# voxelmorph/voxelmorph

Measured on NVIDIA H100. Metric: vol-pairs/sec (3D 160x192x224 VxmDense int_steps=7 train step, NCC+Grad, Adam), higher is better.
Workload: dtype bf16 (conv operands) / f32 (accumulate, warp, VecInt, losses)

## Files before the change

### voxelmorph_b200/csrc/conv3d_tc_wgrad2.cu

```cuda
#include <stdlib.h>

#include <type_traits>

#include "tc_common.cuh"

namespace vxm {
namespace tcw {

using namespace vxm::tc;

constexpr int TH = 4, TWR = 32, TUSE = 30;
constexpr int XROWS = (TH + 2) * TWR;
constexpr int GPAD = 16, GROWS = TH * TWR, GSROWS = GROWS + 2 * GPAD;
constexpr int MAXSLOT = 8, NGS = 4;
constexpr int NLOADER = 128, NTHREADS = 384;

struct Wgrad2Args {
  const __nv_bfloat16* x; int Cx, up, upd;
  const __nv_bfloat16* gz; int Cg;
  float* partial;
  float* bias_partial;
  int B, D, H, W;
  int tiles_h, tiles_w, dchunk, nchunks, nitems, nslot;
  int dbg;
  int xpitch, gpitch;
};

__host__ __device__ inline uint32_t swz(uint32_t off, uint32_t width) { return off ^ (((off >> 7) & (width / 16 - 1)) << 4); }

template <int WIDTH>
__device__ __forceinline__ uint64_t make_desc_mn_swz(uint32_t saddr, uint32_t lbo_bytes) {
  uint64_t d = 0;
  d |= (uint64_t)((saddr >> 4) & 0x3FFF);
  d |= (uint64_t)((lbo_bytes >> 4) & 0x3FFF) << 16;
  d |= (uint64_t)(((8u * WIDTH) >> 4) & 0x3FFF) << 32;
  return d | desc_swizzle(WIDTH);
}

template <int KD, int G, int GOUT, bool KHM = false>
__global__ void __launch_bounds__(NTHREADS, 1) wgrad2_kernel(const Wgrad2Args a) {
  static_assert(!KHM || (KD == 1 && G == 16), "kh-in-M needs a 2-D operand with 16-channel rows");
  constexpr int WA = 2 * G, WG = 2 * GOUT;
  constexpr uint32_t XSLAB = XROWS * WA, GSLAB = GSROWS * WG;
  constexpr int MM = (KD * G > 64) ? 128 : 64;
  constexpr int NN = 3 * GOUT;
  constexpr int NMIRROR = KD == 3 ? 2 : 0, NPADSLAB = KD == 3 ? 1 : 0;
  constexpr int T = KD * 9;
  constexpr int KX = XROWS * (G / 8) / NLOADER, KG = GROWS * (GOUT / 8) / NLOADER;
  static_assert(XROWS * (G / 8) % NLOADER == 0 && GROWS * (GOUT / 8) % NLOADER == 0, "loader tables");
  constexpr int NPART = KHM ? 1 : 2;
  constexpr int NKH = KHM ? 1 : (MM == 128 ? 3 : 2);

  extern __shared__ __align__(1024) uint8_t smem[];
  const int NS = a.nslot;
  uint8_t* s_x = smem;
  uint8_t* s_g = s_x + (size_t)(NS + NMIRROR + NPADSLAB) * XSLAB;
  uint64_t* bars = reinterpret_cast<uint64_t*>(s_g + NGS * GSLAB);
  uint64_t* xfull = bars;
  uint64_t* xempty = bars + MAXSLOT;
  uint64_t* gfull = bars + 2 * MAXSLOT;
  uint64_t* gempty = gfull + NGS;
  float* s_bsum = reinterpret_cast<float*>(bars) + 128;

  const int warp = threadIdx.x >> 5, lane = threadIdx.x & 31;

  for (uint32_t i = threadIdx.x * 16u; i < NGS * GSLAB; i += NTHREADS * 16u) *reinterpret_cast<uint4*>(s_g + i) = make_uint4(0u, 0u, 0u, 0u);
  if (NPADSLAB)
    for (uint32_t i = threadIdx.x * 16u; i < XSLAB; i += NTHREADS * 16u)
      *reinterpret_cast<uint4*>(s_x + (size_t)(NS + NMIRROR) * XSLAB + i) = make_uint4(0u, 0u, 0u, 0u);
  fence_proxy_async();
  if (threadIdx.x == 0) {
    for (int i = 0; i < NS; ++i) { mbar_init(&xfull[i], NLOADER); mbar_init(&xempty[i], 4 * NPART); }
    for (int i = 0; i < NGS; ++i) { mbar_init(&gfull[i], NLOADER); mbar_init(&gempty[i], 4 * NPART); }
    fence_barrier_init();
  }
  __syncthreads();
  const int HW_tiles = a.tiles_h * a.tiles_w;
  const bool has_work = blockIdx.x < a.nitems;

  if (warp >= 8) {
    setmaxnreg_dec<64>();
    const int lt = threadIdx.x - 8 * 32;
    uint32_t xslot = 0, xphase = 1, gslot = 0, gphase = 1;
    const int Dx = a.upd ? a.D >> 1 : a.D, Hx = a.up ? a.H >> 1 : a.H, Wx = a.up ? a.W >> 1 : a.W;
    const int ncx = a.Cx >> 3, ncg = a.Cg >> 3;
    for (int item = blockIdx.x; item < a.nitems; item += gridDim.x) {
      const int wt = item % a.tiles_w, ht = (item / a.tiles_w) % a.tiles_h;
      const int ch = (item / HW_tiles) % a.nchunks, b = item / (HW_tiles * a.nchunks);
      const int h0 = ht * TH, w0 = wt * TUSE, d0 = ch * a.dchunk, d1 = min(d0 + a.dchunk, a.D);
      const int s_begin = KD == 3 ? d0 - 1 : d0, s_end = KD == 3 ? d1 + 1 : d1;
      int soff[KX];
      uint32_t doff[KX];
#pragma unroll
      for (int k = 0; k < KX; ++k) {
        const int id = lt + k * NLOADER;
        const int c8 = id % (G / 8), row = id / (G / 8);
        const int h = h0 - 1 + (row >> 5), w = w0 - 1 + (row & 31);
        doff[k] = swz((uint32_t)row * WA + (uint32_t)c8 * 16u, WA);
        soff[k] = -1;
        if (h >= 0 && h < a.H && w >= 0 && w < a.W && c8 < ncx) soff[k] = ((a.up ? h >> 1 : h) * Wx + (a.up ? w >> 1 : w)) * a.xpitch + c8 * 8;
      }
      int goff[KG];
      uint32_t gdoff[KG];
#pragma unroll
      for (int k = 0; k < KG; ++k) {
        const int id = lt + k * NLOADER;
        const int c8 = id % (GOUT / 8), row = id / (GOUT / 8);
        const int jj = row & 31, h = h0 + (row >> 5), w = w0 - 1 + jj;
        gdoff[k] = swz((uint32_t)(GPAD + row) * WG + (uint32_t)c8 * 16u, WG);
        goff[k] = -1;
        if (jj >= 1 && jj <= TUSE && h < a.H && w < a.W && c8 < ncg) goff[k] = (h * a.W + w) * a.gpitch + c8 * 8;
      }
      for (int ds = s_begin; ds < s_end; ++ds) {
        mbar_wait(&xempty[xslot], xphase);
        uint8_t* slab = s_x + (size_t)xslot * XSLAB;
        const bool dok = ds >= 0 && ds < a.D;
        const __nv_bfloat16* base = a.x + (((size_t)b * Dx + (dok ? (a.upd ? ds >> 1 : ds) : 0)) * Hx * Wx) * a.xpitch;
#pragma unroll
        for (int k = 0; k < KX; ++k) {
          const bool ok = dok && soff[k] >= 0;
          const __nv_bfloat16* src = ok ? base + soff[k] : a.x;
          if (a.dbg & 2) continue;
          cp_async16(slab + doff[k], src, ok ? 16u : 0u);
          if (NMIRROR && xslot < (uint32_t)NMIRROR) cp_async16(slab + (size_t)NS * XSLAB + doff[k], src, ok ? 16u : 0u);
        }
        cp_async_arrive_noinc(&xfull[xslot]);
        if (++xslot == (uint32_t)NS) { xslot = 0; xphase ^= 1; }
        const int dg = KD == 3 ? ds - 1 : ds;
        if (dg >= d0 && dg < d1) {
          mbar_wait(&gempty[gslot], gphase);
          uint8_t* gt = s_g + (size_t)gslot * GSLAB;
          const __nv_bfloat16* baseG = a.gz + (((size_t)b * a.D + dg) * a.H * a.W) * a.gpitch;
#pragma unroll
          for (int k = 0; k < KG; ++k) {
            const bool ok = goff[k] >= 0;
            if (a.dbg & 2) continue;
            cp_async16(gt + gdoff[k], ok ? baseG + goff[k] : a.gz, ok ? 16u : 0u);
          }
          cp_async_arrive_noinc(&gfull[gslot]);
          if (++gslot == NGS) { gslot = 0; gphase ^= 1; }
        }
      }
    }
  } else {
    setmaxnreg_inc<216>();
    const int wg = warp >> 2;
    const int t = threadIdx.x & 127;
    float acc[NKH][NN / 2];
    float* bsum = s_bsum + t * (GOUT + 1);
    if (wg == 0)
#pragma unroll
      for (int c = 0; c < GOUT; ++c) bsum[c] = 0.f;
    const bool do_bias = wg == 0 && a.bias_partial && !(a.dbg & 4);
    uint32_t roff[GOUT / 8];
#pragma unroll
    for (int c8 = 0; c8 < GOUT / 8; ++c8) roff[c8] = swz((uint32_t)(GPAD + t) * WG + (uint32_t)c8 * 16u, WG);
    if (has_work && wg < NPART) {
      const uint32_t x_u32 = smem_u32(s_x), g_u32 = smem_u32(s_g);
      uint32_t wslot = 0, wphase = 0;
      uint32_t hslot = 0;
      uint32_t gs = 0, gph = 0;
      uint32_t acc0 = 0;
      const uint32_t m_off = (MM == 128 && wg == 1) ? 2u * XSLAB : 0u;
      for (int item = blockIdx.x; item < a.nitems; item += gridDim.x) {
        const int ch = (item / HW_tiles) % a.nchunks;
        const int nd = min(ch * a.dchunk + a.dchunk, a.D) - ch * a.dchunk;
        for (int j = 0; j < nd; ++j) {
          const int nwait = (KD == 3 && j == 0) ? 3 : 1;
          for (int q = 0; q < nwait; ++q) {
            mbar_wait(&xfull[wslot], wphase);
            if (++wslot == (uint32_t)NS) { wslot = 0; wphase ^= 1; }
          }
          mbar_wait(&gfull[gs], gph);
          const uint32_t a_start = x_u32 + hslot * XSLAB + m_off;
          const uint32_t b_start = g_u32 + gs * GSLAB + (uint32_t)(GPAD - 1) * WG;
          const uint64_t adesc0 = make_desc_mn_swz<WA>(a_start, KHM ? (uint32_t)(TWR * WA) : (KD == 3 ? XSLAB : 0u));
          const uint64_t bdesc0 = make_desc_mn_swz<WG>(b_start, (uint32_t)WG);
          auto chain = [&](auto nk, int kh0) {
            constexpr int NK = decltype(nk)::value;
            wg_fence();
#pragma unroll
            for (int s = 0; s < NK; ++s) {
#pragma unroll
              for (int i = 0; i < GROWS / 16; ++i) {
                const uint64_t adesc = adesc0 + (uint64_t)((((kh0 + s) * TWR + 16 * i) * WA) >> 4);
                const uint64_t bdesc = bdesc0 + (uint64_t)((16 * i * WG) >> 4);
                Wgmma<NN, 1, 1>::mma(acc[s], adesc, bdesc, i == 0 ? acc0 : 1u);
              }
            }
            wg_commit();
          };
          if (MM == 128 || KHM || wg == 0) chain(std::integral_constant<int, NKH>{}, 0);
          else chain(std::integral_constant<int, 1>{}, 2);
          if (do_bias) {
            const uint8_t* gt = s_g + (size_t)gs * GSLAB;
#pragma unroll
            for (int c8 = 0; c8 < GOUT / 8; ++c8) {
              const uint4 q = *reinterpret_cast<const uint4*>(gt + roff[c8]);
              const __nv_bfloat162* hq = reinterpret_cast<const __nv_bfloat162*>(&q);
#pragma unroll
              for (int e = 0; e < 4; ++e) {
                const float2 f = __bfloat1622float2(hq[e]);
                bsum[c8 * 8 + 2 * e] += f.x;
                bsum[c8 * 8 + 2 * e + 1] += f.y;
              }
            }
          }
          wg_wait<0>();
          if (lane == 0) {
            mbar_arrive(&xempty[hslot]);
            mbar_arrive(&gempty[gs]);
          }
          acc0 = 1u;
          if (++hslot == (uint32_t)NS) hslot = 0;
          if (++gs == NGS) { gs = 0; gph ^= 1; }
        }
        if (KD == 3) {
          if (lane == 0) {
            mbar_arrive(&xempty[hslot]);
            mbar_arrive(&xempty[hslot + 1 == (uint32_t)NS ? 0 : hslot + 1]);
          }
          hslot = hslot + 2 >= (uint32_t)NS ? hslot + 2 - NS : hslot + 2;
        }
      }
    }
    float* part = a.partial + (size_t)blockIdx.x * T * G * GOUT;
    if (!has_work) {
      if (wg == 0)
        for (int i = t; i < T * G * GOUT; i += 128) part[i] = 0.f;
    } else if (wg < NPART) {
      const int w4 = t >> 5, qr = lane >> 2, pc = lane & 3;
#pragma unroll
      for (int s = 0; s < NKH; ++s) {
        const int kh = KHM ? 0 : (MM == 128 ? s : (wg == 0 ? s : 2));
        if (MM != 128 && !KHM && wg == 1 && s > 0) break;
#pragma unroll
        for (int i = 0; i < 2; ++i) {
          const int m = (MM == 128 ? 64 * wg : 0) + 16 * w4 + 8 * i + qr;
          const int kd = KHM ? 0 : m / G, ci = m % G, khm = KHM ? m / G : kh;
          if (kd >= KD || khm >= 3) continue;
#pragma unroll
          for (int jn = 0; jn < NN / 8; ++jn) {
            const int n = 8 * jn + 2 * pc, q = n / GOUT, co = n % GOUT;
            const int tap = (kd * 3 + khm) * 3 + (2 - q);
            *reinterpret_cast<float2*>(part + ((size_t)tap * G + ci) * GOUT + co) = make_float2(acc[s][4 * jn + 2 * i], acc[s][4 * jn + 2 * i + 1]);
          }
        }
      }
    }
    if (wg == 0 && a.bias_partial) {
      named_bar(1, 128);
      if (t < GOUT) {
        float sum = 0.f;
        for (int r2 = 0; r2 < 128; ++r2) sum += s_bsum[r2 * (GOUT + 1) + t];
        a.bias_partial[(size_t)blockIdx.x * GOUT + t] = sum;
      }
    }
  }
}

constexpr int PTH = 2, PTU = 31;
constexpr int PXROWS = (PTH + 1) * TWR, PXR = PXROWS + 8;
constexpr int PGROWS = PTH * TWR;
constexpr uint32_t PXSLAB = PXR * 64, PGSLAB = PGROWS * 64, PGSTAGE = 16 * PGSLAB;
constexpr int PFROWS = 2 * PTH + 1, PFCOLS = 2 * TWR + 1, PFCHUNKS = PFROWS * PFCOLS * 4;
constexpr uint32_t PFSLICE = PFCHUNKS * 16;
constexpr int PNGS = 2, PNSLOT = 4, PMAXSLOT = 8, PNTHREADS = 512;
constexpr size_t PSMEM = (size_t)PNGS * PGSTAGE + 512 + (size_t)PNSLOT * PXSLAB + 3 * PFSLICE + 512 + 128 * 8 * sizeof(float);

struct Wgrad2PolyArgs {
  const __nv_bfloat16* x; int xpitch;
  const __nv_bfloat16* gz; int Cg, gpitch;
  float* partial;
  float* bias_partial;
  int B, D, H, W, Dc, Hc, Wc;
  int tiles_h, tiles_w, dchunk, nchunks, nitems, nslot;
};

__host__ __device__ constexpr int poly_slab(int hl, int ad, int ah, int aw) { return ((hl * 2 + ad) * 2 + ah) * 2 + aw; }

__global__ void __launch_bounds__(PNTHREADS, 1) wgrad2_poly_kernel(const Wgrad2PolyArgs a) {
  extern __shared__ __align__(1024) uint8_t smem[];
  const int NS = a.nslot;
  uint8_t* s_g = smem;
  uint8_t* s_x = s_g + PNGS * PGSTAGE + 512;
  uint8_t* s_f = s_x + (size_t)NS * PXSLAB;
  uint64_t* bars = reinterpret_cast<uint64_t*>(s_f + 3 * PFSLICE);
  uint64_t* xfull = bars;
  uint64_t* xempty = bars + PMAXSLOT;
  uint64_t* gfull = bars + 2 * PMAXSLOT;
  uint64_t* gempty = gfull + PNGS;
  float* s_bsum = reinterpret_cast<float*>(bars) + 128;

  const int warp = threadIdx.x >> 5, lane = threadIdx.x & 31;
  for (uint32_t i = threadIdx.x * 16u; i < (uint32_t)(PNGS * PGSTAGE + 512 + NS * PXSLAB); i += PNTHREADS * 16u)
    *reinterpret_cast<uint4*>(smem + i) = make_uint4(0u, 0u, 0u, 0u);
  fence_proxy_async();
  if (threadIdx.x == 0) {
    for (int i = 0; i < NS; ++i) { mbar_init(&xfull[i], 128); mbar_init(&xempty[i], 12); }
    for (int i = 0; i < PNGS; ++i) { mbar_init(&gfull[i], 128); mbar_init(&gempty[i], 12); }
    fence_barrier_init();
  }
  __syncthreads();
  const int HW_tiles = a.tiles_h * a.tiles_w;
  const bool has_work = blockIdx.x < a.nitems;

  if (warp >= 12) {
    const int lt = threadIdx.x - 12 * 32;
    const int c8 = lt & 3;
    uint32_t xslot = 0, xphase = 1, gslot = 0, gphase = 1;
    float* bsum = s_bsum + lt * 8;
#pragma unroll
    for (int e = 0; e < 8; ++e) bsum[e] = 0.f;
    const bool cok = c8 * 8 < a.Cg;
    for (int item = blockIdx.x; item < a.nitems; item += gridDim.x) {
      const int wt = item % a.tiles_w, ht = (item / a.tiles_w) % a.tiles_h;
      const int ch = (item / HW_tiles) % a.nchunks, b = item / (HW_tiles * a.nchunks);
      const int h0 = ht * PTH, w0 = wt * PTU, d0 = ch * a.dchunk, d1 = min(d0 + a.dchunk, a.Dc + 1);
      constexpr int KX = PXROWS * 4 / 128;
      int soff[KX];
      uint32_t doff[KX];
#pragma unroll
      for (int k = 0; k < KX; ++k) {
        const int row = (lt + k * 128) >> 2;
        const int h = h0 - 1 + row / TWR, w = w0 - 1 + row % TWR;
        doff[k] = swz((uint32_t)row * 64u + (uint32_t)c8 * 16u, 64);
        soff[k] = (h >= 0 && h < a.Hc && w >= 0 && w < a.Wc) ? (h * a.Wc + w) * a.xpitch + c8 * 8 : -1;
      }
      auto load_fine = [&](int f, bool need) {
        if (need) {
          uint8_t* dst = s_f + (size_t)((f + 3) % 3) * PFSLICE;
          const bool fok = f >= 0 && f < a.D;
          for (int idx = lt; idx < PFCHUNKS; idx += 128) {
            const int r = idx / (PFCOLS * 4), rem = idx - r * (PFCOLS * 4), col = rem >> 2, cc = rem & 3;
            const int fh = 2 * h0 - 1 + r, fw = 2 * w0 - 3 + col;
            const bool ok = fok && fh >= 0 && fh < a.H && fw >= 0 && fw < a.W && cc * 8 < a.Cg;
            cp_async16(dst + (size_t)idx * 16, ok ? a.gz + ((((size_t)b * a.D + f) * a.H + fh) * a.W + fw) * a.gpitch + cc * 8 : a.gz,
                       ok ? 16u : 0u);
          }
        }
        cp_async_commit();
      };
      load_fine(2 * d0 - 1, true);
      load_fine(2 * d0, true);
      load_fine(2 * d0 + 1, true);
      for (int s = d0 - 1; s < d1; ++s) {
        mbar_wait(&xempty[xslot], xphase);
        uint8_t* slab = s_x + (size_t)xslot * PXSLAB;
        const bool dok = s >= 0 && s < a.Dc;
        const __nv_bfloat16* base = a.x + ((size_t)b * a.Dc + (dok ? s : 0)) * a.Hc * a.Wc * a.xpitch;
#pragma unroll
        for (int k = 0; k < KX; ++k) {
          const bool ok = dok && soff[k] >= 0;
          cp_async16(slab + doff[k], ok ? base + soff[k] : a.x, ok ? 16u : 0u);
        }
        cp_async_arrive_noinc(&xfull[xslot]);
        if (++xslot == (uint32_t)NS) { xslot = 0; xphase ^= 1; }
        if (s < d0) continue;
        mbar_wait(&gempty[gslot], gphase);
        uint8_t* st = s_g + (size_t)gslot * PGSTAGE;
#pragma unroll 1
        for (int ad = 0; ad < 2; ++ad) {
          cp_async_wait<1>();
          named_bar(1, 128);
#pragma unroll 1
          for (int u = lt >> 2; u < PGROWS; u += 32) {
            const int i = u / TWR, j = u % TWR;
            float g[2][2][8];
#pragma unroll
            for (int q = 0; q < 32; ++q) (&g[0][0][0])[q] = 0.f;
            if (j > 0 && cok) {
#pragma unroll
              for (int kd = 0; kd < 2; ++kd) {
                const int fd = 2 * s - 1 + ad + kd;
                if (fd < 0 || fd >= a.D) continue;
                const uint8_t* fs = s_f + (size_t)((fd + 3) % 3) * PFSLICE;
#pragma unroll
                for (int kh = 0; kh < 3; ++kh) {
                  float f[3][8];
#pragma unroll
                  for (int kw = 0; kw < 3; ++kw) {
                    const uint4 q = *reinterpret_cast<const uint4*>(fs + (size_t)((((2 * i + kh) * PFCOLS) + 2 * j + kw) * 4 + c8) * 16);
                    const __nv_bfloat162* hq = reinterpret_cast<const __nv_bfloat162*>(&q);
#pragma unroll
                    for (int e = 0; e < 4; ++e) {
                      const float2 v = __bfloat1622float2(hq[e]);
                      f[kw][2 * e] = v.x; f[kw][2 * e + 1] = v.y;
                    }
                  }
#pragma unroll
                  for (int ah = 0; ah < 2; ++ah) {
                    if (ah == 0 ? kh == 2 : kh == 0) continue;
#pragma unroll
                    for (int e = 0; e < 8; ++e) {
                      g[ah][0][e] += f[0][e] + f[1][e];
                      g[ah][1][e] += f[1][e] + f[2][e];
                    }
                  }
                }
              }
              if (ad == 1)
#pragma unroll
                for (int e = 0; e < 8; ++e) bsum[e] += g[1][1][e];
            }
            const uint32_t roff = swz((uint32_t)u * 64u + (uint32_t)c8 * 16u, 64);
#pragma unroll
            for (int ah = 0; ah < 2; ++ah)
#pragma unroll
              for (int aw = 0; aw < 2; ++aw) {
                uint32_t hi[4], lo[4];
#pragma unroll
                for (int e = 0; e < 4; ++e) {
                  const float v0 = g[ah][aw][2 * e], v1 = g[ah][aw][2 * e + 1];
                  const __nv_bfloat162 h2 = __floats2bfloat162_rn(v0, v1);
                  const float2 hf = __bfloat1622float2(h2);
                  hi[e] = *reinterpret_cast<const uint32_t*>(&h2);
                  lo[e] = pack_bf16x2(v0 - hf.x, v1 - hf.y);
                }
                *reinterpret_cast<uint4*>(st + (size_t)poly_slab(0, ad, ah, aw) * PGSLAB + roff) = make_uint4(hi[0], hi[1], hi[2], hi[3]);
                *reinterpret_cast<uint4*>(st + (size_t)poly_slab(1, ad, ah, aw) * PGSLAB + roff) = make_uint4(lo[0], lo[1], lo[2], lo[3]);
              }
          }
          named_bar(1, 128);
          load_fine(2 * s + 2 + ad, s + 1 < d1);
        }
        fence_proxy_async();
        mbar_arrive(&gfull[gslot]);
        if (++gslot == PNGS) { gslot = 0; gphase ^= 1; }
      }
    }
    if (a.bias_partial) {
      named_bar(1, 128);
      if (lt < 32) {
        float sum = 0.f;
        for (int r = 0; r < 32; ++r) sum += s_bsum[(4 * r + (lt >> 3)) * 8 + (lt & 7)];
        a.bias_partial[(size_t)blockIdx.x * 32 + lt] = has_work ? sum : 0.f;
      }
    }
  } else {
    const int wg = warp >> 2;
    const int t = threadIdx.x & 127;
    const int ad = wg == 1 ? 1 : 0;
    float acc[3][32];
    if (has_work) {
      const uint32_t x_u32 = smem_u32(s_x), g_u32 = smem_u32(s_g);
      uint32_t wslot = 0, wphase = 0, hslot = 0, gs = 0, gph = 0, acc0 = 0;
      for (int item = blockIdx.x; item < a.nitems; item += gridDim.x) {
        const int ch = (item / HW_tiles) % a.nchunks;
        const int nd = min(ch * a.dchunk + a.dchunk, a.Dc + 1) - ch * a.dchunk;
        for (int j = 0; j < nd; ++j) {
          for (int q = 0; q < (j == 0 ? 2 : 1); ++q) {
            mbar_wait(&xfull[wslot], wphase);
            if (++wslot == (uint32_t)NS) { wslot = 0; wphase ^= 1; }
          }
          mbar_wait(&gfull[gs], gph);
          const uint32_t cur = hslot + 1 == (uint32_t)NS ? 0 : hslot + 1;
          const uint32_t a_base = x_u32 + (wg == 0 ? hslot : cur) * PXSLAB;
          const uint32_t b_base = g_u32 + gs * PGSTAGE + 64u;
          wg_fence();
#pragma unroll
          for (int s3 = 0; s3 < 3; ++s3) {
            const int ah = s3 == 1 ? 1 : 0;
            const uint64_t adesc0 = make_desc_mn_swz<64>(a_base + (s3 == 0 ? 0u : (uint32_t)TWR * 64u), 64u);
#pragma unroll
            for (int i = 0; i < PGROWS / 16; ++i)
#pragma unroll
              for (int hl = 0; hl < 2; ++hl) {
                const uint64_t adesc = adesc0 + (uint64_t)((16 * i * 64) >> 4);
                const uint64_t bdesc = make_desc_mn_swz<64>(b_base + (uint32_t)poly_slab(hl, ad, ah, 0) * PGSLAB + 16u * i * 64u, PGSLAB);
                Wgmma<64, 1, 1>::mma(acc[s3], adesc, bdesc, (i == 0 && hl == 0) ? acc0 : 1u);
              }
          }
          wg_commit();
          wg_wait<0>();
          if (lane == 0) {
            mbar_arrive(&xempty[hslot]);
            mbar_arrive(&gempty[gs]);
          }
          acc0 = 1u;
          hslot = cur;
          if (++gs == PNGS) { gs = 0; gph ^= 1; }
        }
        if (lane == 0) mbar_arrive(&xempty[hslot]);
        if (++hslot == (uint32_t)NS) hslot = 0;
      }
    }
    float* part = a.partial + (size_t)blockIdx.x * 27 * 32 * 32;
    if (!has_work) {
      for (int i = threadIdx.x; i < 27 * 32 * 32; i += 384) part[i] = 0.f;
    } else {
      const int w4 = t >> 5, qr = lane >> 2, pc = lane & 3;
#pragma unroll
      for (int s3 = 0; s3 < 3; ++s3)
#pragma unroll
        for (int i = 0; i < 2; ++i) {
          const int m = 16 * w4 + 8 * i + qr, sw = m >> 5, ci = m & 31;
#pragma unroll
          for (int jn = 0; jn < 8; ++jn) {
            const int n = 8 * jn + 2 * pc, aw = n >> 5, co = n & 31;
            if (sw == 0 && aw == 1) continue;
            const int kw = aw == 1 ? 1 : (sw == 0 ? 0 : 2);
            const int tap = (wg * 3 + s3) * 3 + kw;
            *reinterpret_cast<float2*>(part + ((size_t)tap * 32 + ci) * 32 + co) = make_float2(acc[s3][4 * jn + 2 * i], acc[s3][4 * jn + 2 * i + 1]);
          }
        }
    }
  }
}

__global__ void __launch_bounds__(256) wgrad2_reduce_kernel(const float* __restrict__ partial, float* __restrict__ gw, int ncta, int T, int G,
                                                            int GOUT, int Cout, int Cin_total, int ci_off, int ci_cnt,
                                                            const float* __restrict__ bias_partial, float* __restrict__ gb, int accumulate) {
  __shared__ float sh[4][64];
  const int tx = threadIdx.x & 63, ty = threadIdx.x >> 6;
  if (gb && blockIdx.x == 0 && threadIdx.x < Cout) {
    float acc = accumulate ? gb[threadIdx.x] : 0.f;
    for (int c = 0; c < ncta; ++c) acc += bias_partial[(size_t)c * GOUT + threadIdx.x];
    gb[threadIdx.x] = acc;
  }
  const int per_cta = T * G * GOUT;
  const int j = blockIdx.x * 64 + tx;
  const int q = (ncta + 3) / 4, c0 = ty * q, c1 = min(c0 + q, ncta);
  float acc = 0.f;
  if (j < per_cta)
    for (int c = c0; c < c1; ++c) acc += partial[(size_t)c * per_cta + j];
  sh[ty][tx] = acc;
  __syncthreads();
  if (ty == 0 && j < per_cta) {
    const int co = j % GOUT, ci = (j / GOUT) % G, tap = j / (GOUT * G);
    if (co < Cout && ci < ci_cnt) {
      const float tot = ((sh[0][tx] + sh[1][tx]) + sh[2][tx]) + sh[3][tx];
      float* dst = gw + ((size_t)co * Cin_total + ci_off + ci) * T + tap;
      *dst = (accumulate ? *dst : 0.f) + tot;
    }
  }
}

struct ReduceDesc {
  const float* partial; float* gw; const float* bias_partial; float* gb;
  int ncta, T, G, GOUT, Cout, Cin_total, ci_off, ci_cnt, accumulate, blk_begin;
  int co_off;
};
constexpr int MAXRED = 40;
struct ReduceBatch {
  ReduceDesc d[MAXRED];
  int n, total_blocks;
};
__global__ void __launch_bounds__(256) wgrad2_reduce_multi_kernel(const ReduceBatch rb) {
  __shared__ float sh[4][64];
  int k = 0;
  for (int i = 1; i < rb.n; ++i)
    if ((int)blockIdx.x >= rb.d[i].blk_begin) k = i;
  const ReduceDesc& r = rb.d[k];
  const int blk = blockIdx.x - r.blk_begin;
  const int tx = threadIdx.x & 63, ty = threadIdx.x >> 6;
  if (r.gb && blk == 0 && threadIdx.x < r.Cout) {
    float acc = r.accumulate ? r.gb[threadIdx.x] : 0.f;
    for (int c = 0; c < r.ncta; ++c) acc += r.bias_partial[(size_t)c * r.GOUT + threadIdx.x];
    r.gb[threadIdx.x] = acc;
  }
  const int per_cta = r.T * r.G * r.GOUT;
  const int j = blk * 64 + tx;
  const int q = (r.ncta + 3) / 4, c0 = ty * q, c1 = min(c0 + q, r.ncta);
  float acc = 0.f;
  if (j < per_cta)
    for (int c = c0; c < c1; ++c) acc += r.partial[(size_t)c * per_cta + j];
  sh[ty][tx] = acc;
  __syncthreads();
  if (ty == 0 && j < per_cta) {
    const int co = j % r.GOUT, ci = (j / r.GOUT) % r.G, tap = j / (r.GOUT * r.G);
    if (co < r.Cout && ci < r.ci_cnt) {
      const float tot = ((sh[0][tx] + sh[1][tx]) + sh[2][tx]) + sh[3][tx];
      float* dst = r.gw + ((size_t)(r.co_off + co) * r.Cin_total + r.ci_off + ci) * r.T + tap;
      *dst = (r.accumulate ? *dst : 0.f) + tot;
    }
  }
}

}
}

using namespace vxm;
using namespace vxm::tcw;

namespace vxm {
namespace tcw {

static bool chan_ok(int c) { return c == 8 || c == 16 || c == 32; }

bool wgrad2_supported(int Ca, int Cb, int Cg) {
  const char* e = getenv("VXM_B200_WGRAD");
  if (e && e[0] == 'o') return false;
  return (Ca == 0 || chan_ok(Ca)) && (Cb == 0 || chan_ok(Cb)) && Ca + Cb > 0 && chan_ok(Cg);
}

static int wgrad2_dchunk(int D, long long tiles, int nsm, double halo) {
  int best_nch = 1;
  double best_cost = 1e300;
  for (int nch = 1; nch <= 32 && nch <= D; ++nch) {
    const int dc = (D + nch - 1) / nch;
    const long long items = tiles * ((D + dc - 1) / dc);
    const long long waves = (items + nsm - 1) / nsm;
    const double cost = (double)waves * (dc + halo);
    if (cost < best_cost - 1e-9) { best_cost = cost; best_nch = nch; }
  }
  return (D + best_nch - 1) / best_nch;
}

static int wgrad2_finish(float* partial, float* bias_partial, int grid, int T, int G, int GOUT, float* grad_w, float* grad_b, int Cout_real,
                         int Cin_total, int ci_off, int ci_cnt, int accumulate, cudaStream_t st, ReduceDesc* defer, int co_off) {
  const int per_cta = T * G * GOUT;
  if (defer) {
    defer->partial = partial; defer->gw = grad_w; defer->bias_partial = bias_partial; defer->gb = grad_b;
    defer->ncta = grid; defer->T = T; defer->G = G; defer->GOUT = GOUT; defer->Cout = Cout_real; defer->Cin_total = Cin_total;
    defer->ci_off = ci_off; defer->ci_cnt = ci_cnt; defer->accumulate = accumulate; defer->blk_begin = (per_cta + 63) / 64;
    defer->co_off = co_off;
    return VXM_OK;
  }
  wgrad2_reduce_kernel<<<(per_cta + 63) / 64, 256, 0, st>>>(partial, grad_w, grid, T, G, GOUT, Cout_real, Cin_total, ci_off, ci_cnt,
                                                              bias_partial, grad_b, accumulate);
  return check_launch("conv3d_tc_wgrad2_reduce");
}

static bool wgrad2_poly_ok(int Cx, int up, int Cg, int kd, int D, int H, int W) {
  const char* e = getenv("VXM_B200_POLYPHASE");
  if (e && e[0] == '0' && e[1] == 0) return false;
  return up && kd == 3 && Cx == 32 && Cg == 32 && D % 2 == 0 && H % 2 == 0 && W % 2 == 0;
}

static int wgrad2_poly_launch(const void* x, int x_pitch, const void* gz, int Cg, int g_pitch, float* grad_w, float* grad_b, void* work, int B,
                              int D, int H, int W, int Cout_real, int Cin_total, int ci_off, int ci_cnt, int accumulate, cudaStream_t st,
                              ReduceDesc* defer, size_t* work_used, int co_off) {
  Wgrad2PolyArgs a{};
  a.x = (const __nv_bfloat16*)x; a.xpitch = x_pitch;
  a.gz = (const __nv_bfloat16*)gz; a.Cg = Cg; a.gpitch = g_pitch;
  a.B = B; a.D = D; a.H = H; a.W = W; a.Dc = D / 2; a.Hc = H / 2; a.Wc = W / 2;
  a.tiles_h = (a.Hc + PTH) / PTH; a.tiles_w = (a.Wc + PTU) / PTU;
  const int nsm = conv_ctas();
  const long long tiles = (long long)B * a.tiles_h * a.tiles_w;
  a.dchunk = wgrad2_dchunk(a.Dc + 1, tiles, nsm, 0.5);
  a.nchunks = (a.Dc + a.dchunk) / a.dchunk;
  a.nitems = (int)(tiles * a.nchunks);
  int grid = a.nitems < nsm ? a.nitems : nsm;
  if (grid > 256) grid = 256;
  a.partial = (float*)work;
  if (defer) {
    const size_t npart = (size_t)grid * 27 * 32 * 32;
    a.bias_partial = grad_b ? (float*)work + npart : nullptr;
    *work_used = (npart + (grad_b ? (size_t)grid * 32 : 0)) * sizeof(float);
    *work_used = (*work_used + 255) & ~(size_t)255;
  } else {
    a.bias_partial = grad_b ? (float*)work + (size_t)256 * 27 * 64 * 32 : nullptr;
  }
  a.nslot = PNSLOT;
  const size_t smem = PSMEM;
  VXM_CUDA(cudaFuncSetAttribute(wgrad2_poly_kernel, cudaFuncAttributeMaxDynamicSharedMemorySize, (int)smem));
  wgrad2_poly_kernel<<<grid, PNTHREADS, smem, st>>>(a);
  int rc = check_launch("conv3d_tc_wgrad2_poly");
  if (rc) return rc;
  return wgrad2_finish(a.partial, a.bias_partial, grid, 27, 32, 32, grad_w, grad_b, Cout_real, Cin_total, ci_off, ci_cnt, accumulate, st, defer,
                       co_off);
}

int wgrad2_launch(const void* x, int Cx, int up, const void* gz, int Cg, float* grad_w, float* grad_b, void* work, int B, int D, int H, int W,
                  int kd, int Cout_real, int Cin_total, int ci_off, int ci_cnt, int accumulate, cudaStream_t st, ReduceDesc* defer,
                  size_t* work_used, bool khm, int x_pitch, int g_pitch, int co_off) {
  VXM_REQUIRE(defer || co_off == 0, "conv3d_tc_wgrad2: gz slices need the deferred reduction");
  if (!khm && wgrad2_poly_ok(Cx, up, Cg, kd, D, H, W))
    return wgrad2_poly_launch(x, x_pitch ? x_pitch : Cx, gz, Cg, g_pitch ? g_pitch : Cg, grad_w, grad_b, work, B, D, H, W, Cout_real, Cin_total,
                              ci_off, ci_cnt, accumulate, st, defer, work_used, co_off);
  Wgrad2Args a{};
  a.x = (const __nv_bfloat16*)x; a.Cx = Cx; a.up = up; a.upd = (up && kd == 3) ? 1 : 0;
  a.gz = (const __nv_bfloat16*)gz; a.Cg = Cg;
  a.xpitch = x_pitch ? x_pitch : Cx; a.gpitch = g_pitch ? g_pitch : Cg;
  a.B = B; a.D = D; a.H = H; a.W = W;
  a.tiles_h = (H + TH - 1) / TH; a.tiles_w = (W + TUSE - 1) / TUSE;
  {
    const char* de = getenv("VXM_B200_WGRAD_DBG");
    a.dbg = de ? atoi(de) : 0;
  }
  const int G = Cx <= 16 ? 16 : 32, GOUT = Cg <= 16 ? 16 : 32;
  const int nsm = conv_ctas();
  const long long tiles = (long long)B * a.tiles_h * a.tiles_w;
  a.dchunk = wgrad2_dchunk(D, tiles, nsm, kd == 3 ? 2.5 : 0.5);
  a.nchunks = (D + a.dchunk - 1) / a.dchunk;
  a.nitems = (int)(tiles * a.nchunks);
  int grid = a.nitems < nsm ? a.nitems : nsm;
  if (grid > 256) grid = 256;
  a.partial = (float*)work;
  if (defer) {
    const size_t npart = (size_t)grid * kd * 9 * G * GOUT;
    a.bias_partial = grad_b ? (float*)work + npart : nullptr;
    *work_used = (npart + (grad_b ? (size_t)grid * GOUT : 0)) * sizeof(float);
    *work_used = (*work_used + 255) & ~(size_t)255;
  } else {
    a.bias_partial = grad_b ? (float*)work + (size_t)256 * kd * 9 * 64 * 32 : nullptr;
  }
  const size_t xslab = (size_t)XROWS * 2 * G, gslab = (size_t)GSROWS * 2 * GOUT;
  const int extra = kd == 3 ? 3 : 0;
  int nslot = (int)((200 * 1024 - NGS * gslab - 512) / xslab) - extra;
  if (nslot > MAXSLOT) nslot = MAXSLOT;
  VXM_REQUIRE(nslot >= 4, "conv3d_tc_wgrad: not enough shared memory for the slab ring");
  a.nslot = nslot;
  const size_t smem = (size_t)(nslot + extra) * xslab + NGS * gslab + 512 + 128 * (GOUT + 1) * sizeof(float);
#define VXM_W2_LAUNCH(KD_, G_, GO_)                                                                                          \
  do {                                                                                                                       \
    VXM_CUDA(cudaFuncSetAttribute(wgrad2_kernel<KD_, G_, GO_>, cudaFuncAttributeMaxDynamicSharedMemorySize, (int)smem));     \
    wgrad2_kernel<KD_, G_, GO_><<<grid, NTHREADS, smem, st>>>(a);                                                             \
  } while (0)
#define VXM_W2_G(KD_)                                                                                                        \
  do {                                                                                                                       \
    if (G == 16 && GOUT == 16) VXM_W2_LAUNCH(KD_, 16, 16); else if (G == 16) VXM_W2_LAUNCH(KD_, 16, 32);                     \
    else if (GOUT == 16) VXM_W2_LAUNCH(KD_, 32, 16); else VXM_W2_LAUNCH(KD_, 32, 32);                                        \
  } while (0)
  if (khm) {
    VXM_REQUIRE(kd == 1 && G == 16 && GOUT == 16 && !up, "conv3d_tc_wgrad2 (kh in M): needs kd = 1 and at most 16 channels on both sides");
    VXM_CUDA(cudaFuncSetAttribute(wgrad2_kernel<1, 16, 16, true>, cudaFuncAttributeMaxDynamicSharedMemorySize, (int)smem));
    wgrad2_kernel<1, 16, 16, true><<<grid, NTHREADS, smem, st>>>(a);
  } else if (kd == 3) VXM_W2_G(3); else VXM_W2_G(1);
  int rc = check_launch("conv3d_tc_wgrad2");
  if (rc) return rc;
  return wgrad2_finish(a.partial, a.bias_partial, grid, kd * 9, G, GOUT, grad_w, grad_b, Cout_real, Cin_total, ci_off, ci_cnt, accumulate, st,
                       defer, co_off);
}

}
}

extern "C" size_t vxm_conv3d_tc_wgrad2_desc_bytes(void) { return sizeof(ReduceDesc); }
extern "C" int vxm_conv3d_tc_wgrad2_max_pending(void) { return MAXRED; }
extern "C" size_t vxm_conv3d_tc_wgrad2_partial_bytes(int kd) {
  return 2 * ((size_t)256 * kd * 9 * 32 * 32 + 256 * 32) * sizeof(float) + 1024;
}

static bool chan_ok64(int c) { return chan_ok(c) || c == 64; }

extern "C" int vxm_conv3d_tc_wgrad2_partial(const void* xa, const void* xb, const void* gz, float* grad_w, float* grad_b, void* work,
                                            size_t work_bytes, size_t* work_used, void* descs_host, int* ndesc, int B, int D, int H, int W,
                                            int Ca, int Cb, int up, int Cin_real, int Cg, int Cout_real, int kd, int accumulate, void* stream) {
  VXM_REQUIRE(B > 0 && D > 0 && H > 0 && W > 0 && grad_w && work && work_used && descs_host && ndesc && gz, "conv3d_tc_wgrad2_partial: bad argument");
  VXM_REQUIRE(kd == 1 || kd == 3, "conv3d_tc_wgrad2_partial: kd must be 1 or 3");
  const char* e = getenv("VXM_B200_WGRAD");
  VXM_REQUIRE(!(e && e[0] == 'o') && (Ca == 0 || chan_ok64(Ca)) && (Cb == 0 || chan_ok64(Cb)) && Ca + Cb > 0 && chan_ok64(Cg),
              "conv3d_tc_wgrad2_partial: channel counts (%d,%d | %d) unsupported", Ca, Cb, Cg);
  VXM_REQUIRE((Ca == 0 || xa) && (Cb == 0 || xb), "conv3d_tc_wgrad2_partial: missing source tensor");
  const int nsub = ((Ca + 31) / 32 + (Cb + 31) / 32) * ((Cg + 31) / 32);
  VXM_REQUIRE(*ndesc + (nsub > 2 ? nsub : 2) <= MAXRED, "conv3d_tc_wgrad2_partial: too many pending reductions (flush first)");
  VXM_REQUIRE(Cout_real > 0 && Cout_real <= Cg, "conv3d_tc_wgrad2_partial: Cout_real out of range");
  ReduceDesc* d = (ReduceDesc*)descs_host;
  cudaStream_t st = as_stream(stream);
  size_t total = 0;
  char* wp = (char*)work;
  const void* src[2] = {xa, xb};
  const int C[2] = {Ca, Cb}, ci0[2] = {0, Ca}, sup[2] = {up, 0};
  for (int s = 0; s < 2; ++s) {
    for (int xs = 0; xs < C[s] && ci0[s] + xs < Cin_real; xs += 32) {
      const int cx = C[s] - xs < 32 ? C[s] - xs : 32;
      const int cnt = Cin_real - ci0[s] - xs < cx ? Cin_real - ci0[s] - xs : cx;
      for (int gs = 0; gs < Cg && gs < Cout_real; gs += 32) {
        const int cg = Cg - gs < 32 ? Cg - gs : 32;
        const int cout = Cout_real - gs < cg ? Cout_real - gs : cg;
        float* gb = (grad_b && ci0[s] + xs == 0) ? grad_b + gs : nullptr;
        size_t used = 0;
        int rc = wgrad2_launch((const __nv_bfloat16*)src[s] + xs, cx, sup[s], (const __nv_bfloat16*)gz + gs, cg, grad_w, gb, wp, B, D, H, W,
                               kd, cout, Cin_real, ci0[s] + xs, cnt, accumulate, st, &d[*ndesc], &used, false, C[s], Cg, gs);
        if (rc) return rc;
        VXM_REQUIRE(total + used <= work_bytes, "conv3d_tc_wgrad2_partial: workspace too small");
        ++*ndesc; wp += used; total += used;
      }
    }
  }
  *work_used = total;
  return VXM_OK;
}

extern "C" int vxm_conv3d_tc_wgrad2_partial_khm(const void* x, const void* gz, float* grad_w, float* grad_b, void* work, size_t work_bytes,
                                                size_t* work_used, void* descs_host, int* ndesc, int B, int D, int H, int W, int Cx,
                                                int Cin_real, int Cg, int Cout_real, int accumulate, void* stream) {
  VXM_REQUIRE(B > 0 && D > 0 && H > 0 && W > 0 && x && gz && grad_w && work && work_used && descs_host && ndesc, "conv3d_tc_wgrad2_partial_khm: bad argument");
  VXM_REQUIRE((Cx == 8 || Cx == 16) && (Cg == 8 || Cg == 16), "conv3d_tc_wgrad2_partial_khm: channel counts (%d | %d) unsupported", Cx, Cg);
  VXM_REQUIRE(Cin_real > 0 && Cin_real <= Cx && Cout_real > 0 && Cout_real <= Cg, "conv3d_tc_wgrad2_partial_khm: real channel counts out of range");
  VXM_REQUIRE(*ndesc + 1 <= MAXRED, "conv3d_tc_wgrad2_partial_khm: too many pending reductions (flush first)");
  ReduceDesc* d = (ReduceDesc*)descs_host;
  size_t used = 0;
  int rc = wgrad2_launch(x, Cx, 0, gz, Cg, grad_w, grad_b, work, B, D, H, W, 1, Cout_real, Cin_real, 0, Cin_real, accumulate, as_stream(stream),
                         &d[*ndesc], &used, true, 0, 0, 0);
  if (rc) return rc;
  VXM_REQUIRE(used <= work_bytes, "conv3d_tc_wgrad2_partial_khm: workspace too small");
  ++*ndesc;
  *work_used = used;
  return VXM_OK;
}

extern "C" int vxm_conv3d_tc_wgrad2_flush(const void* descs_host, int ndesc, void* stream) {
  VXM_REQUIRE(descs_host && ndesc > 0 && ndesc <= MAXRED, "conv3d_tc_wgrad2_flush: bad argument");
  ReduceBatch rb;
  const ReduceDesc* d = (const ReduceDesc*)descs_host;
  int blocks = 0;
  for (int i = 0; i < ndesc; ++i) {
    rb.d[i] = d[i];
    const int nb = d[i].blk_begin;
    rb.d[i].blk_begin = blocks;
    blocks += nb;
  }
  rb.n = ndesc; rb.total_blocks = blocks;
  wgrad2_reduce_multi_kernel<<<blocks, 256, 0, as_stream(stream)>>>(rb);
  return check_launch("conv3d_tc_wgrad2_reduce_multi");
}
```

Before: 79.26.

## Rework polyphase wgrad producer with TMA loads, fine-slice ring and carried sums

The polyphase weight-gradient kernel now loads the coarse activations and fine gradient slices with TMA 5D tensor maps. Fine slices go into a four-slot mbarrier ring fed by a single producer thread, replacing per-thread cp.async loops. The gradient precompute reuses partial depth sums across passes through a carry register array, so each fine slice is folded in once rather than twice. The MMA warpgroups now wait with one wgmma group in flight before releasing slots, the g stage count rises to three, and the tile height drops to one row. These changes add register pressure and more tiles per volume, and the code now depends on TMA zero-fill handling the boundaries correctly.

New measurement: 80.85 (median of 6 runs). +2.0%, better.

```diff
diff --git a/voxelmorph_b200/csrc/conv3d_tc_wgrad2.cu b/voxelmorph_b200/csrc/conv3d_tc_wgrad2.cu
--- a/voxelmorph_b200/csrc/conv3d_tc_wgrad2.cu
+++ b/voxelmorph_b200/csrc/conv3d_tc_wgrad2.cu
@@ -259,46 +259,57 @@
   }
 }
 
-constexpr int PTH = 2, PTU = 31;
+constexpr int PTH = 1, PTU = 31;
 constexpr int PXROWS = (PTH + 1) * TWR, PXR = PXROWS + 8;
 constexpr int PGROWS = PTH * TWR;
 constexpr uint32_t PXSLAB = PXR * 64, PGSLAB = PGROWS * 64, PGSTAGE = 16 * PGSLAB;
-constexpr int PFROWS = 2 * PTH + 1, PFCOLS = 2 * TWR + 1, PFCHUNKS = PFROWS * PFCOLS * 4;
-constexpr uint32_t PFSLICE = PFCHUNKS * 16;
-constexpr int PNGS = 2, PNSLOT = 4, PMAXSLOT = 8, PNTHREADS = 512;
-constexpr size_t PSMEM = (size_t)PNGS * PGSTAGE + 512 + (size_t)PNSLOT * PXSLAB + 3 * PFSLICE + 512 + 128 * 8 * sizeof(float);
+constexpr int PFROWS = 2 * PTH + 1, PFCOLS = 2 * PTU + 3;
+constexpr uint32_t PFBYTES = PFROWS * PFCOLS * 64;
+constexpr int PNGS = 3, PNSLOT = 4, PNFS = 4, PMAXSLOT = 8, PNTHREADS = 512;
+constexpr uint32_t PXSTRIDE = (PXSLAB + 1023) & ~1023u, PFSTRIDE = (PFBYTES + 1023) & ~1023u;
+constexpr uint32_t PXOFF = ((uint32_t)PNGS * PGSTAGE + 512 + 1023) & ~1023u;
+constexpr uint32_t PFOFF = PXOFF + PNSLOT * PXSTRIDE, PBOFF = PFOFF + PNFS * PFSTRIDE;
+static_assert(PFSTRIDE >= (PFROWS * PFCOLS + 1) * 64, "fine slot padding");
+constexpr size_t PSMEM = PBOFF + 512 + 128 * 8 * sizeof(float);
+static_assert(PSMEM <= 232448, "wgrad2_poly_kernel: shared memory");
 
 struct Wgrad2PolyArgs {
-  const __nv_bfloat16* x; int xpitch;
-  const __nv_bfloat16* gz; int Cg, gpitch;
   float* partial;
   float* bias_partial;
   int B, D, H, W, Dc, Hc, Wc;
-  int tiles_h, tiles_w, dchunk, nchunks, nitems, nslot;
+  int tiles_h, tiles_w, dchunk, nchunks, nitems;
+  alignas(64) CUtensorMap tmx, tmg;
 };
 
 __host__ __device__ constexpr int poly_slab(int hl, int ad, int ah, int aw) { return ((hl * 2 + ad) * 2 + ah) * 2 + aw; }
 
-__global__ void __launch_bounds__(PNTHREADS, 1) wgrad2_poly_kernel(const Wgrad2PolyArgs a) {
+__device__ __forceinline__ float2 bf2_at(const uint4& q, int e) {
+  const uint32_t w = e == 0 ? q.x : (e == 1 ? q.y : (e == 2 ? q.z : q.w));
+  return __bfloat1622float2(*reinterpret_cast<const __nv_bfloat162*>(&w));
+}
+
+__global__ void __launch_bounds__(PNTHREADS, 1) wgrad2_poly_kernel(const __grid_constant__ Wgrad2PolyArgs a) {
   extern __shared__ __align__(1024) uint8_t smem[];
-  const int NS = a.nslot;
+  constexpr int NS = PNSLOT;
   uint8_t* s_g = smem;
-  uint8_t* s_x = s_g + PNGS * PGSTAGE + 512;
-  uint8_t* s_f = s_x + (size_t)NS * PXSLAB;
-  uint64_t* bars = reinterpret_cast<uint64_t*>(s_f + 3 * PFSLICE);
+  uint8_t* s_x = smem + PXOFF;
+  uint8_t* s_f = smem + PFOFF;
+  uint64_t* bars = reinterpret_cast<uint64_t*>(smem + PBOFF);
   uint64_t* xfull = bars;
   uint64_t* xempty = bars + PMAXSLOT;
   uint64_t* gfull = bars + 2 * PMAXSLOT;
   uint64_t* gempty = gfull + PNGS;
+  uint64_t* ffull = gempty + PNGS;
+  uint64_t* fempty = ffull + PNFS;
   float* s_bsum = reinterpret_cast<float*>(bars) + 128;
 
   const int warp = threadIdx.x >> 5, lane = threadIdx.x & 31;
-  for (uint32_t i = threadIdx.x * 16u; i < (uint32_t)(PNGS * PGSTAGE + 512 + NS * PXSLAB); i += PNTHREADS * 16u)
-    *reinterpret_cast<uint4*>(smem + i) = make_uint4(0u, 0u, 0u, 0u);
+  for (uint32_t i = threadIdx.x * 16u; i < PBOFF; i += PNTHREADS * 16u) *reinterpret_cast<uint4*>(smem + i) = make_uint4(0u, 0u, 0u, 0u);
   fence_proxy_async();
   if (threadIdx.x == 0) {
-    for (int i = 0; i < NS; ++i) { mbar_init(&xfull[i], 128); mbar_init(&xempty[i], 12); }
+    for (int i = 0; i < NS; ++i) { mbar_init(&xfull[i], 1); mbar_init(&xempty[i], 12); }
     for (int i = 0; i < PNGS; ++i) { mbar_init(&gfull[i], 128); mbar_init(&gempty[i], 12); }
+    for (int i = 0; i < PNFS; ++i) { mbar_init(&ffull[i], 1); mbar_init(&fempty[i], 4); }
     fence_barrier_init();
   }
   __syncthreads();
@@ -307,123 +318,112 @@
 
   if (warp >= 12) {
     const int lt = threadIdx.x - 12 * 32;
-    const int c8 = lt & 3;
+    const int c8 = lt & 3, j = lt >> 2;
+    const int rs = j > 0 ? PFCOLS : 0, cs = j > 0 ? 1 : 0, c0 = j > 0 ? 2 * j : PFROWS * PFCOLS;
+    const bool producer = lt == 0;
     uint32_t xslot = 0, xphase = 1, gslot = 0, gphase = 1;
     float* bsum = s_bsum + lt * 8;
 #pragma unroll
     for (int e = 0; e < 8; ++e) bsum[e] = 0.f;
-    const bool cok = c8 * 8 < a.Cg;
+    if (producer) {
+      tma_prefetch_desc(&a.tmx);
+      tma_prefetch_desc(&a.tmg);
+    }
+    uint32_t pslot = 0, pphase = 1;
+    int pitem = blockIdx.x, pk = 0;
+    auto produce_fine = [&]() {
+      if (pitem >= a.nitems) return;
+      const int wt = pitem % a.tiles_w, ht = (pitem / a.tiles_w) % a.tiles_h;
+      const int ch = (pitem / HW_tiles) % a.nchunks, b = pitem / (HW_tiles * a.nchunks);
+      const int d0 = ch * a.dchunk, d1 = min(d0 + a.dchunk, a.Dc + 1);
+      mbar_wait(&fempty[pslot], pphase);
+      mbar_expect_tx(&ffull[pslot], PFBYTES);
+      tma_load_5d(s_f + pslot * PFSTRIDE, &a.tmg, 0, 2 * wt * PTU - 3, 2 * ht * PTH - 1, 2 * d0 - 1 + pk, b, &ffull[pslot]);
+      if (++pslot == PNFS) { pslot = 0; pphase ^= 1; }
+      if (++pk == 2 * (d1 - d0) + 1) { pk = 0; pitem += gridDim.x; }
+    };
+    auto produce_x = [&](int s, int h0, int w0, int b) {
+      mbar_wait(&xempty[xslot], xphase);
+      mbar_expect_tx(&xfull[xslot], PXROWS * 64);
+      tma_load_5d(s_x + xslot * PXSTRIDE, &a.tmx, 0, w0 - 1, h0 - 1, s, b, &xfull[xslot]);
+      if (++xslot == (uint32_t)NS) { xslot = 0; xphase ^= 1; }
+    };
+    if (producer)
+      for (int k = 0; k < PNFS; ++k) produce_fine();
+    uint32_t cslot = 0, cphase = 0;
+    float carry[PTH][2][2][8];
+    auto pass = [&](auto adc, uint8_t* st) {
+      constexpr int AD = decltype(adc)::value;
+      mbar_wait(&ffull[cslot], cphase);
+      const uint8_t* fs = s_f + cslot * PFSTRIDE;
+#pragma unroll
+      for (int i = 0; i < PTH; ++i) {
+        float p[2][2][8];
+        uint4 q[3][3];
+#pragma unroll
+        for (int kh = 0; kh < 3; ++kh)
+#pragma unroll
+          for (int kw = 0; kw < 3; ++kw)
+            q[kh][kw] = *reinterpret_cast<const uint4*>(fs + swz((uint32_t)(((2 * i + kh) * rs + c0 + kw * cs) * 64 + c8 * 16), 64));
+#pragma unroll
+        for (int kh = 0; kh < 3; ++kh) {
+#pragma unroll
+          for (int e2 = 0; e2 < 4; ++e2) {
+            const float2 f0 = bf2_at(q[kh][0], e2), f1 = bf2_at(q[kh][1], e2), f2 = bf2_at(q[kh][2], e2);
+            const float o[2] = {f0.x + f1.x, f0.y + f1.y}, ev[2] = {f1.x + f2.x, f1.y + f2.y};
+#pragma unroll
+            for (int h = 0; h < 2; ++h) {
+              const int e = 2 * e2 + h;
+              if (kh == 0) { p[0][0][e] = o[h]; p[0][1][e] = ev[h]; }
+              if (kh == 1) { p[0][0][e] += o[h]; p[0][1][e] += ev[h]; p[1][0][e] = o[h]; p[1][1][e] = ev[h]; }
+              if (kh == 2) { p[1][0][e] += o[h]; p[1][1][e] += ev[h]; }
+            }
+          }
+        }
+        if (AD >= 0) {
+          const uint32_t roff = swz((uint32_t)(i * TWR + j) * 64u + (uint32_t)c8 * 16u, 64);
+#pragma unroll
+          for (int ah = 0; ah < 2; ++ah)
+#pragma unroll
+            for (int aw = 0; aw < 2; ++aw) {
+              float g[8];
+#pragma unroll
+              for (int e = 0; e < 8; ++e) g[e] = carry[i][ah][aw][e] + p[ah][aw][e];
+              if (AD == 1 && ah == 1 && aw == 1)
+#pragma unroll
+                for (int e = 0; e < 8; ++e) bsum[e] += g[e];
+              uint32_t hi[4], lo[4];
+#pragma unroll
+              for (int e = 0; e < 4; ++e) {
+                const __nv_bfloat162 h2 = __floats2bfloat162_rn(g[2 * e], g[2 * e + 1]);
+                const float2 hf = __bfloat1622float2(h2);
+                hi[e] = *reinterpret_cast<const uint32_t*>(&h2);
+                lo[e] = pack_bf16x2(g[2 * e] - hf.x, g[2 * e + 1] - hf.y);
+              }
+              *reinterpret_cast<uint4*>(st + (size_t)poly_slab(0, AD, ah, aw) * PGSLAB + roff) = make_uint4(hi[0], hi[1], hi[2], hi[3]);
+              *reinterpret_cast<uint4*>(st + (size_t)poly_slab(1, AD, ah, aw) * PGSLAB + roff) = make_uint4(lo[0], lo[1], lo[2], lo[3]);
+            }
+        }
+#pragma unroll
+        for (int q = 0; q < 32; ++q) (&carry[i][0][0][0])[q] = (&p[0][0][0])[q];
+      }
+      __syncwarp();
+      if (lane == 0) mbar_arrive(&fempty[cslot]);
+      if (++cslot == PNFS) { cslot = 0; cphase ^= 1; }
+      if (producer) produce_fine();
+    };
     for (int item = blockIdx.x; item < a.nitems; item += gridDim.x) {
       const int wt = item % a.tiles_w, ht = (item / a.tiles_w) % a.tiles_h;
       const int ch = (item / HW_tiles) % a.nchunks, b = item / (HW_tiles * a.nchunks);
       const int h0 = ht * PTH, w0 = wt * PTU, d0 = ch * a.dchunk, d1 = min(d0 + a.dchunk, a.Dc + 1);
-      constexpr int KX = PXROWS * 4 / 128;
-      int soff[KX];
-      uint32_t doff[KX];
-#pragma unroll
-      for (int k = 0; k < KX; ++k) {
-        const int row = (lt + k * 128) >> 2;
-        const int h = h0 - 1 + row / TWR, w = w0 - 1 + row % TWR;
-        doff[k] = swz((uint32_t)row * 64u + (uint32_t)c8 * 16u, 64);
-        soff[k] = (h >= 0 && h < a.Hc && w >= 0 && w < a.Wc) ? (h * a.Wc + w) * a.xpitch + c8 * 8 : -1;
-      }
-      auto load_fine = [&](int f, bool need) {
-        if (need) {
-          uint8_t* dst = s_f + (size_t)((f + 3) % 3) * PFSLICE;
-          const bool fok = f >= 0 && f < a.D;
-          for (int idx = lt; idx < PFCHUNKS; idx += 128) {
-            const int r = idx / (PFCOLS * 4), rem = idx - r * (PFCOLS * 4), col = rem >> 2, cc = rem & 3;
-            const int fh = 2 * h0 - 1 + r, fw = 2 * w0 - 3 + col;
-            const bool ok = fok && fh >= 0 && fh < a.H && fw >= 0 && fw < a.W && cc * 8 < a.Cg;
-            cp_async16(dst + (size_t)idx * 16, ok ? a.gz + ((((size_t)b * a.D + f) * a.H + fh) * a.W + fw) * a.gpitch + cc * 8 : a.gz,
-                       ok ? 16u : 0u);
-          }
-        }
-        cp_async_commit();
-      };
-      load_fine(2 * d0 - 1, true);
-      load_fine(2 * d0, true);
-      load_fine(2 * d0 + 1, true);
-      for (int s = d0 - 1; s < d1; ++s) {
-        mbar_wait(&xempty[xslot], xphase);
-        uint8_t* slab = s_x + (size_t)xslot * PXSLAB;
-        const bool dok = s >= 0 && s < a.Dc;
-        const __nv_bfloat16* base = a.x + ((size_t)b * a.Dc + (dok ? s : 0)) * a.Hc * a.Wc * a.xpitch;
-#pragma unroll
-        for (int k = 0; k < KX; ++k) {
-          const bool ok = dok && soff[k] >= 0;
-          cp_async16(slab + doff[k], ok ? base + soff[k] : a.x, ok ? 16u : 0u);
-        }
-        cp_async_arrive_noinc(&xfull[xslot]);
-        if (++xslot == (uint32_t)NS) { xslot = 0; xphase ^= 1; }
-        if (s < d0) continue;
+      if (producer) produce_x(d0 - 1, h0, w0, b);
+      pass(std::integral_constant<int, -1>{}, nullptr);
+      for (int s = d0; s < d1; ++s) {
         mbar_wait(&gempty[gslot], gphase);
+        if (producer) produce_x(s, h0, w0, b);
         uint8_t* st = s_g + (size_t)gslot * PGSTAGE;
-#pragma unroll 1
-        for (int ad = 0; ad < 2; ++ad) {
-          cp_async_wait<1>();
-          named_bar(1, 128);
-#pragma unroll 1
-          for (int u = lt >> 2; u < PGROWS; u += 32) {
-            const int i = u / TWR, j = u % TWR;
-            float g[2][2][8];
-#pragma unroll
-            for (int q = 0; q < 32; ++q) (&g[0][0][0])[q] = 0.f;
-            if (j > 0 && cok) {
-#pragma unroll
-              for (int kd = 0; kd < 2; ++kd) {
-                const int fd = 2 * s - 1 + ad + kd;
-                if (fd < 0 || fd >= a.D) continue;
-                const uint8_t* fs = s_f + (size_t)((fd + 3) % 3) * PFSLICE;
-#pragma unroll
-                for (int kh = 0; kh < 3; ++kh) {
-                  float f[3][8];
-#pragma unroll
-                  for (int kw = 0; kw < 3; ++kw) {
-                    const uint4 q = *reinterpret_cast<const uint4*>(fs + (size_t)((((2 * i + kh) * PFCOLS) + 2 * j + kw) * 4 + c8) * 16);
-                    const __nv_bfloat162* hq = reinterpret_cast<const __nv_bfloat162*>(&q);
-#pragma unroll
-                    for (int e = 0; e < 4; ++e) {
-                      const float2 v = __bfloat1622float2(hq[e]);
-                      f[kw][2 * e] = v.x; f[kw][2 * e + 1] = v.y;
-                    }
-                  }
-#pragma unroll
-                  for (int ah = 0; ah < 2; ++ah) {
-                    if (ah == 0 ? kh == 2 : kh == 0) continue;
-#pragma unroll
-                    for (int e = 0; e < 8; ++e) {
-                      g[ah][0][e] += f[0][e] + f[1][e];
-                      g[ah][1][e] += f[1][e] + f[2][e];
-                    }
-                  }
-                }
-              }
-              if (ad == 1)
-#pragma unroll
-                for (int e = 0; e < 8; ++e) bsum[e] += g[1][1][e];
-            }
-            const uint32_t roff = swz((uint32_t)u * 64u + (uint32_t)c8 * 16u, 64);
-#pragma unroll
-            for (int ah = 0; ah < 2; ++ah)
-#pragma unroll
-              for (int aw = 0; aw < 2; ++aw) {
-                uint32_t hi[4], lo[4];
-#pragma unroll
-                for (int e = 0; e < 4; ++e) {
-                  const float v0 = g[ah][aw][2 * e], v1 = g[ah][aw][2 * e + 1];
-                  const __nv_bfloat162 h2 = __floats2bfloat162_rn(v0, v1);
-                  const float2 hf = __bfloat1622float2(h2);
-                  hi[e] = *reinterpret_cast<const uint32_t*>(&h2);
-                  lo[e] = pack_bf16x2(v0 - hf.x, v1 - hf.y);
-                }
-                *reinterpret_cast<uint4*>(st + (size_t)poly_slab(0, ad, ah, aw) * PGSLAB + roff) = make_uint4(hi[0], hi[1], hi[2], hi[3]);
-                *reinterpret_cast<uint4*>(st + (size_t)poly_slab(1, ad, ah, aw) * PGSLAB + roff) = make_uint4(lo[0], lo[1], lo[2], lo[3]);
-              }
-          }
-          named_bar(1, 128);
-          load_fine(2 * s + 2 + ad, s + 1 < d1);
-        }
+        pass(std::integral_constant<int, 0>{}, st);
+        pass(std::integral_constant<int, 1>{}, st);
         fence_proxy_async();
         mbar_arrive(&gfull[gslot]);
         if (++gslot == PNGS) { gslot = 0; gphase ^= 1; }
@@ -445,6 +445,7 @@
     if (has_work) {
       const uint32_t x_u32 = smem_u32(s_x), g_u32 = smem_u32(s_g);
       uint32_t wslot = 0, wphase = 0, hslot = 0, gs = 0, gph = 0, acc0 = 0;
+      uint32_t ph = 0, pg = 0;
       for (int item = blockIdx.x; item < a.nitems; item += gridDim.x) {
         const int ch = (item / HW_tiles) % a.nchunks;
         const int nd = min(ch * a.dchunk + a.dchunk, a.Dc + 1) - ch * a.dchunk;
@@ -455,7 +456,7 @@
           }
           mbar_wait(&gfull[gs], gph);
           const uint32_t cur = hslot + 1 == (uint32_t)NS ? 0 : hslot + 1;
-          const uint32_t a_base = x_u32 + (wg == 0 ? hslot : cur) * PXSLAB;
+          const uint32_t a_base = x_u32 + (wg == 0 ? hslot : cur) * PXSTRIDE;
           const uint32_t b_base = g_u32 + gs * PGSTAGE + 64u;
           wg_fence();
 #pragma unroll
@@ -472,16 +473,22 @@
               }
           }
           wg_commit();
-          wg_wait<0>();
-          if (lane == 0) {
-            mbar_arrive(&xempty[hslot]);
-            mbar_arrive(&gempty[gs]);
-          }
+          wg_wait<1>();
+          if (j > 0 && lane == 0) {
+            mbar_arrive(&xempty[ph]);
+            mbar_arrive(&gempty[pg]);
+          }
+          ph = hslot; pg = gs;
           acc0 = 1u;
           hslot = cur;
           if (++gs == PNGS) { gs = 0; gph ^= 1; }
         }
-        if (lane == 0) mbar_arrive(&xempty[hslot]);
+        wg_wait<0>();
+        if (lane == 0) {
+          mbar_arrive(&xempty[ph]);
+          mbar_arrive(&gempty[pg]);
+          mbar_arrive(&xempty[hslot]);
+        }
         if (++hslot == (uint32_t)NS) hslot = 0;
       }
     }
@@ -628,13 +635,14 @@
   return up && kd == 3 && Cx == 32 && Cg == 32 && D % 2 == 0 && H % 2 == 0 && W % 2 == 0;
 }
 
-static int wgrad2_poly_launch(const void* x, int x_pitch, const void* gz, int Cg, int g_pitch, float* grad_w, float* grad_b, void* work, int B,
+static int wgrad2_poly_launch(const void* x, int x_pitch, const void* gz, int g_pitch, float* grad_w, float* grad_b, void* work, int B,
                               int D, int H, int W, int Cout_real, int Cin_total, int ci_off, int ci_cnt, int accumulate, cudaStream_t st,
                               ReduceDesc* defer, size_t* work_used, int co_off) {
   Wgrad2PolyArgs a{};
-  a.x = (const __nv_bfloat16*)x; a.xpitch = x_pitch;
-  a.gz = (const __nv_bfloat16*)gz; a.Cg = Cg; a.gpitch = g_pitch;
   a.B = B; a.D = D; a.H = H; a.W = W; a.Dc = D / 2; a.Hc = H / 2; a.Wc = W / 2;
+  if (tc::make_act_tmap(&a.tmx, x, B, a.Dc, a.Hc, a.Wc, x_pitch, 32, TWR, PTH + 1) != 0 ||
+      tc::make_act_tmap(&a.tmg, gz, B, D, H, W, g_pitch, 32, PFCOLS, PFROWS) != 0)
+    return VXM_ERR_CUDA;
   a.tiles_h = (a.Hc + PTH) / PTH; a.tiles_w = (a.Wc + PTU) / PTU;
   const int nsm = conv_ctas();
   const long long tiles = (long long)B * a.tiles_h * a.tiles_w;
@@ -652,7 +660,6 @@
   } else {
     a.bias_partial = grad_b ? (float*)work + (size_t)256 * 27 * 64 * 32 : nullptr;
   }
-  a.nslot = PNSLOT;
   const size_t smem = PSMEM;
   VXM_CUDA(cudaFuncSetAttribute(wgrad2_poly_kernel, cudaFuncAttributeMaxDynamicSharedMemorySize, (int)smem));
   wgrad2_poly_kernel<<<grid, PNTHREADS, smem, st>>>(a);
@@ -667,7 +674,7 @@
                   size_t* work_used, bool khm, int x_pitch, int g_pitch, int co_off) {
   VXM_REQUIRE(defer || co_off == 0, "conv3d_tc_wgrad2: gz slices need the deferred reduction");
   if (!khm && wgrad2_poly_ok(Cx, up, Cg, kd, D, H, W))
-    return wgrad2_poly_launch(x, x_pitch ? x_pitch : Cx, gz, Cg, g_pitch ? g_pitch : Cg, grad_w, grad_b, work, B, D, H, W, Cout_real, Cin_total,
+    return wgrad2_poly_launch(x, x_pitch ? x_pitch : Cx, gz, g_pitch ? g_pitch : Cg, grad_w, grad_b, work, B, D, H, W, Cout_real, Cin_total,
                               ci_off, ci_cnt, accumulate, st, defer, work_used, co_off);
   Wgrad2Args a{};
   a.x = (const __nv_bfloat16*)x; a.Cx = Cx; a.up = up; a.upd = (up && kd == 3) ? 1 : 0;
```
